# mfkiwl/conan-slam

Hardware: AMD Instinct MI355X
Metric: ekf_update_steps_per_sec (higher is better)
Workload: dtype f32

## Files before the change

conan_slam_amd/csrc/cslam_ekf.hip:

```cpp
#include <hip/hip_runtime.h>

#include <algorithm>
#include <atomic>
#include <cfloat>
#include <cmath>
#include <cstdint>
#include <cstdlib>
#include <new>
#include <string>
#include <thread>
#include <vector>

#include "cslam_common.hpp"
#include "ekf_kernels.hpp"
#include "ekf_kernels_fast.hpp"
#include "ekf_landmark_kernels.hpp"
#include "ekf_lookahead.hpp"
#include "ekf_pgemm_limbs.hpp"
#include "ekf_pose_kernels.hpp"
#include "host_linalg.hpp"

namespace cslam
{
__global__ void ekf_la_signal_kernel(unsigned* signal, unsigned add)
{
    if (threadIdx.x == 0)
    {
        atomicAdd(signal, add);
    }
}
__global__ void __launch_bounds__(128) ekf_la_wide_f32(LaWideArgs a)
{
    ekf_la_wide_body<1, 0>(a);
}
__global__ void __launch_bounds__(128) ekf_la_wide_f32_k64(LaWideArgs a)
{
    ekf_la_wide_body<1, 64>(a);
}
}

using namespace cslam;

namespace
{

std::atomic<int>& g_engines = ::cslam::live_engines();

constexpr int    kStagingSlots = 64;
constexpr size_t kLdsBudget    = 150 * 1024;

struct EkfBase
{
    virtual ~EkfBase() {}
    int         dtype    = CSLAM_F32;
    int         fuse_f64 = 1;
    int         pgemm_limbs_req = -1, limbs_kmin_req = -1;
    int         xcd_queues_req = -1;
    int         device   = 0;
    int         quirks   = CSLAM_Q_REF_EXACT;
    int         nmax     = 0;
    int         ncap     = 0;
    int         ldp      = 0;
    int         n        = 3;
    int         sync_mode = 1;
    int         seq_defer     = 1;
    int         lower         = 0;
    int         pipeline      = 0;
    int         pgemm_spare   = 16;
    int         gather_corr_wide = 1;
    int         pgemm_wgs     = 0;
    int         lookahead     = -1;
    hipStream_t stream   = nullptr;
    hipStream_t stream_b = nullptr;
    long long   la_windows = 0;

    virtual int init()                                                                        = 0;
    virtual int set_state(const void* X, int n, const void* P, int ldp)                        = 0;
    virtual int get_state(void* X, void* P, int ldp)                                           = 0;
    virtual int get_x(void* X, int cap)                                                        = 0;
    virtual int get_landmarks(int first, int count, void* x, void* pll, void* pvl)             = 0;
    virtual int trace(double* tr)                                                              = 0;
    virtual int predict(double v, double swa, const void* Q, double wb, double dt)             = 0;
    virtual int update(const void* Z, int m, const void* R, const int* idf, int batch, bool on_device) = 0;
    virtual int augment(const void* Z, int q, const void* R)                                   = 0;
    virtual int observe_heading(double phi, int use)                                           = 0;
    virtual int associate(const void* Z, int m, const void* R, double g1, double g2, int* idf_out, int* kind) = 0;
    virtual int factor_status(int* flags, int clear)                                           = 0;
    virtual int set_profiling(int on)                                                          = 0;
    virtual int get_stage_times(double* ms, int* launches)                                     = 0;
    virtual int debug_last_update(void* PHT, void* S, void* G, void* W1, void* V, int* k)      = 0;
    virtual int set_deferred(int max_cols)                                                     = 0;
    virtual int do_flush()                                                                     = 0;
    virtual int resolve_predict()                                                              = 0;
    virtual void set_fuse_predict(int on)                                                      = 0;
    virtual int sync_all()                                                                     = 0;
    virtual int la_drain()                                                                     = 0;
};

template <typename T>
struct Ekf : EkfBase
{
    T*   dX = nullptr;
    T*   dP = nullptr;
    T*   dPv = nullptr;
    T*   dWv = nullptr;
    int* dPoseDone = nullptr;
    int* dSign     = nullptr;
    T*   dLm       = nullptr;
    int  hd_cols[2] = {0, 0};
    int        wcur = 0;
    unsigned   inflight_mask = 0;
    hipEvent_t ev_a2b = nullptr, ev_pgemm = nullptr;
    T*         last_slot = nullptr;
    int  kcap  = 0;
    T*   dPHT  = nullptr;
    T*   dW1   = nullptr;
    T*   dY    = nullptr;
    int  wcap  = 0;
    int  kp    = 0;
    int  defer_max = 0;
    T*   dS    = nullptr;
    T*   dG    = nullptr;
    T*   dSub  = nullptr;
    T*   dM    = nullptr;
    bool m_valid = false;
    bool g_from_gt  = false;
    bool sub_valid = false;
    T*   dGt   = nullptr;
    T*   dV    = nullptr;
    T*   dt_   = nullptr;
    T*   dU    = nullptr;
    T*   dScrS = nullptr;
    T*   dScrG = nullptr;
    int* dFlags = nullptr;
    int* hFlags = nullptr;
    T* dHead = nullptr;
    int         mcap   = 0;
    void*       hStage = nullptr;
    void*       dStage = nullptr;
    hipEvent_t  stage_ev[kStagingSlots];
    bool        stage_ev_used[kStagingSlots];
    int         stage_next = 0;
    int*       dTicket     = nullptr;
    int        pgemm_limbs = 0;
    int        xcd_queues  = 0;
    int        limbs_kmin  = 65;
    uint4*     dWb         = nullptr;
    size_t     wb_bytes    = 0;
    int2*      dTilesM     = nullptr;
    int*       dSegOff     = nullptr;
    int*       dTicketX    = nullptr;
    int        tilesM_built = 0;
    int        limb_parity = 0;
    unsigned   launch_parity = 0;
    int        psym_nt = -1;
    int2* dTiles      = nullptr;
    int   tiles_built = 0;
    int   n_sym_tiles = 0;
    int   num_cus     = 256;
    int sticky_host = 0;
    int last_k      = 0;
    int kp_call_limit = 0;
    int                     profiling = 0;
    unsigned                prof_count = 0;
    bool                    prof_sampled = false;
    std::vector<hipEvent_t> ev_pool;
    std::vector<int>        ev_stage;
    size_t                  ev_used = 0;

    ~Ekf() override
    {
        if (stream)
        {
            (void)hipStreamSynchronize(stream);
        }
        if (stream_b && stream_b != stream)
        {
            (void)hipStreamSynchronize(stream_b);
        }
        if (stream_f)
        {
            (void)hipStreamSynchronize(stream_f);
            (void)hipEventDestroy(ev_fb);
            (void)hipEventDestroy(ev_raw);
            (void)hipStreamDestroy(stream_f);
        }
        la_free();
        if (ev_a2b)
        {
            (void)hipEventDestroy(ev_a2b);
        }
        if (ev_pgemm)
        {
            (void)hipEventDestroy(ev_pgemm);
// ... 25 lines not shown
        (void)hipFree(dSegOff);
        (void)hipFree(dTicketX);
        (void)hipFree(dPred);
        (void)hipFree(dAssoc);
        (void)hipFree(dAssocOut);
        (void)hipFree(dW1);
        (void)hipFree(dY);
        (void)hipFree(dTiles);
        (void)hipFree(dStage);
        if (hStage)
        {
            (void)hipHostFree(hStage);
        }
        if (hFlags)
        {
            (void)hipHostFree(hFlags);
        }
        if (stream_b && stream_b != stream)
        {
            (void)hipStreamDestroy(stream_b);
        }
        if (stream)
        {
            (void)hipStreamDestroy(stream);
        }
    }

    T* wbase(int region) const { return dW1 + (size_t)region * wcap * ldp; }

    void free_workspace()
    {
        (void)hipFree(dPHT);
        (void)hipFree(dS);
        (void)hipFree(dG);
        (void)hipFree(dSub);
        (void)hipFree(dM);
        dM = nullptr;
        (void)hipFree(dGt);
        (void)hipFree(dV);
        (void)hipFree(dt_);
        (void)hipFree(dU);
        (void)hipFree(dScrS);
        (void)hipFree(dScrG);
        dPHT = dS = dG = dSub = dGt = dV = dt_ = dU = dScrS = dScrG = nullptr;
    }

    int use_device() { CSLAM_HIP_TRY(hipSetDevice(device)); return CSLAM_OK; }

    int init() override
    {
        for (int i = 0; i < kStagingSlots; i++)
        {
            stage_ev_used[i] = false;
        }
        int rc = use_device();
        if (rc)
        {
            return rc;
        }
        if (xcd_queues_req >= 0)
        {
            xcd_queues = xcd_queues_req;
        }
        if (pgemm_limbs_req >= 0)
        {
            pgemm_limbs = (pgemm_limbs_req == 6 || pgemm_limbs_req == 9) ? pgemm_limbs_req : 0;
        }
        if (limbs_kmin_req >= 0)
        {
            limbs_kmin = std::max(57, limbs_kmin_req);
        }
        if (pipeline)
        {
            int lo = 0, hi = 0;
            CSLAM_HIP_TRY(hipDeviceGetStreamPriorityRange(&lo, &hi));
            CSLAM_HIP_TRY(hipStreamCreateWithPriority(&stream, hipStreamNonBlocking, hi));
            CSLAM_HIP_TRY(hipStreamCreateWithPriority(&stream_b, hipStreamNonBlocking, lo));
        }
        else
        {
            CSLAM_HIP_TRY(hipStreamCreateWithFlags(&stream, hipStreamNonBlocking));
            stream_b = stream;
        }
        CSLAM_HIP_TRY(hipEventCreateWithFlags(&ev_a2b, hipEventDisableTiming));
        CSLAM_HIP_TRY(hipEventCreateWithFlags(&ev_pgemm, hipEventDisableTiming));
        {
            hipDeviceProp_t prop;
            CSLAM_HIP_TRY(hipGetDeviceProperties(&prop, device));
            num_cus = prop.multiProcessorCount > 0 ? prop.multiProcessorCount : 256;
        }
        size_t pbytes = (size_t)ldp * ldp * sizeof(T);
        CSLAM_HIP_TRY(hipMalloc(&dX, (size_t)ldp * sizeof(T)));
        CSLAM_HIP_TRY(hipMalloc(&dP, pbytes));
        CSLAM_HIP_TRY(hipMemsetAsync(dX, 0, (size_t)ldp * sizeof(T), stream));
        CSLAM_HIP_TRY(hipMemsetAsync(dP, 0, pbytes, stream));
        CSLAM_HIP_TRY(hipMalloc(&dPv, (size_t)3 * ldp * sizeof(T)));
        CSLAM_HIP_TRY(hipMemsetAsync(dPv, 0, (size_t)3 * ldp * sizeof(T), stream));
        CSLAM_HIP_TRY(hipMalloc(&dPoseDone, 4 * sizeof(int)));
        CSLAM_HIP_TRY(hipMemsetAsync(dPoseDone, 0, 4 * sizeof(int), stream));
        CSLAM_HIP_TRY(hipMalloc(&dFlags, 2 * sizeof(int)));
        CSLAM_HIP_TRY(hipMemsetAsync(dFlags, 0, 2 * sizeof(int), stream));
        CSLAM_HIP_TRY(hipHostMalloc(&hFlags, 2 * sizeof(int), hipHostMallocDefault));
        CSLAM_HIP_TRY(hipMalloc(&dHead, ((size_t)3 * ldp + 2) * sizeof(T)));
        CSLAM_HIP_TRY(hipMemsetAsync(dHead, 0, ((size_t)3 * ldp + 2) * sizeof(T), stream));
        CSLAM_HIP_TRY(hipFuncSetAttribute(reinterpret_cast<const void*>(&ekf_factor_kernel<T>),
                                          hipFuncAttributeMaxDynamicSharedMemorySize, 160 * 1024));
        if (sizeof(T) == 4)
        {
            CSLAM_HIP_TRY(hipFuncSetAttribute(reinterpret_cast<const void*>(&ekf_factor_mfma_big_f32<128>),
                                              hipFuncAttributeMaxDynamicSharedMemorySize, 160 * 1024));
        }
        else
        {
            CSLAM_HIP_TRY(hipFuncSetAttribute(reinterpret_cast<const void*>(&ekf_factor_mfma_f64<64>),
                                              hipFuncAttributeMaxDynamicSharedMemorySize, 160 * 1024));
            CSLAM_HIP_TRY(hipFuncSetAttribute(reinterpret_cast<const void*>(&ekf_factor_mfma_f64<32>),
                                              hipFuncAttributeMaxDynamicSharedMemorySize, 160 * 1024));
            CSLAM_HIP_TRY(hipFuncSetAttribute(reinterpret_cast<const void*>(&ekf_downdate_f64<4>),
                                              hipFuncAttributeMaxDynamicSharedMemorySize, 160 * 1024));
            CSLAM_HIP_TRY(hipFuncSetAttribute(reinterpret_cast<const void*>(&ekf_downdate_f64<2>),
                                              hipFuncAttributeMaxDynamicSharedMemorySize, 160 * 1024));
        }
        CSLAM_HIP_TRY(hipMalloc(&dTicket, 2 * sizeof(int)));
        CSLAM_HIP_TRY(hipMemsetAsync(dTicket, 0, 2 * sizeof(int), stream));
        if (const char* sv = getenv("CSLAM_LA_K64"))
        {
            la_k64 = atoi(sv) ? 1 : 0;
        }
        if (const char* sv = getenv("CSLAM_LA_WG_SIGNAL"))
        {
            la_wg_signal = atoi(sv) ? 1 : 0;
        }
        if (const char* sv = getenv("CSLAM_PSYM_NT"))
        {
            psym_nt = atoi(sv) ? 1 : 0;
        }
        rc = ensure_k(64);
        if (rc)
        {
            return rc;
        }
        rc = ensure_w(128);
        if (rc)
        {
            return rc;
        }
        rc = ensure_m(64);
        if (rc)
        {
            return rc;
        }
        CSLAM_HIP_TRY(hipStreamSynchronize(stream));
        return CSLAM_OK;
    }

    int ensure_k(int k)
    {
        if (k <= kcap)
        {
            return CSLAM_OK;
        }
        int newk = round_up(std::max(k, 2 * kcap), 8);
        CSLAM_HIP_TRY(hipStreamSynchronize(stream));
        free_workspace();
        size_t pan = (size_t)ldp * newk * sizeof(T);
        size_t kk  = (size_t)newk * (newk + 1) * sizeof(T);
        CSLAM_HIP_TRY(hipMalloc(&dPHT, pan));
        CSLAM_HIP_TRY(hipMalloc(&dS, kk));
        CSLAM_HIP_TRY(hipMalloc(&dG, kk));
        if (dSub == nullptr)
        {
            CSLAM_HIP_TRY(hipMalloc(&dSub, (size_t)(3 + 64) * 64 * sizeof(T)));
            CSLAM_HIP_TRY(hipMalloc(&dM, (size_t)3 * 128 * sizeof(T)));
        }
        CSLAM_HIP_TRY(hipMalloc(&dGt, kk));
        CSLAM_HIP_TRY(hipMalloc(&dScrS, kk));
        CSLAM_HIP_TRY(hipMalloc(&dScrG, kk));
        CSLAM_HIP_TRY(hipMalloc(&dV, (size_t)newk * sizeof(T)));
        CSLAM_HIP_TRY(hipMalloc(&dt_, (size_t)newk * sizeof(T)));
        CSLAM_HIP_TRY(hipMalloc(&dU, (size_t)newk * sizeof(T)));
        CSLAM_HIP_TRY(hipMemsetAsync(dPHT, 0, pan, stream));
        (void)hipFree(dWv);
        dWv = nullptr;
        CSLAM_HIP_TRY(hipMalloc(&dWv, (size_t)3 * newk * sizeof(T)));
        CSLAM_HIP_TRY(hipMemsetAsync(dWv, 0, (size_t)3 * newk * sizeof(T), stream));
// ... 201 lines not shown
    int launch_negcol_fix(T* W, int kcols, hipStream_t st)
    {
        const int tiles = round_up(n, kTile) / kTile;
        int       rc    = CSLAM_OK;
        if (lower && (rc = ensure_tile_list(tiles)))
        {
            return rc;
        }
        const int nt = lower ? n_sym_tiles : tiles * tiles;
        hipLaunchKernelGGL(ekf_negcol_fix_kernel<T>, dim3(std::min(nt, 2 * num_cus)), dim3(256), 0, st, dP, ldp, n, W, ldp,
                           kcols, dSign + (size_t)wcur * wcap, dSign + (size_t)2 * wcap + wcur,
                           lower ? dTiles : (const int2*)nullptr, nt, tiles, dPoseDone + 2, (stream_b == stream) ? 1 : 0);
        CSLAM_HIP_TRY(hipGetLastError());
        return CSLAM_OK;
    }

    int flush_wait()
    {
        int rc = flush();
        return rc ? rc : wait_pgemm();
    }

    size_t slot_bytes(int mc) const { return (size_t)mc * (2 * sizeof(T) + sizeof(int)); }

    int ensure_m(int m)
    {
        if (m <= mcap)
        {
            return CSLAM_OK;
        }
        int newm = std::max(m, 2 * mcap);
        if (int rc = la_drain())
        {
            return rc;
        }
        CSLAM_HIP_TRY(hipStreamSynchronize(stream));
        if (stream_f)
        {
            CSLAM_HIP_TRY(hipStreamSynchronize(stream_f));
        }
        if (hStage)
        {
            (void)hipHostFree(hStage);
            hStage = nullptr;
        }
        (void)hipFree(dStage);
        dStage = nullptr;
        CSLAM_HIP_TRY(hipHostMalloc(&hStage, slot_bytes(newm) * kStagingSlots, hipHostMallocDefault));
        CSLAM_HIP_TRY(hipMalloc(&dStage, slot_bytes(newm) * kStagingSlots));
        mcap = newm;
        return CSLAM_OK;
    }

    int stage_obs(const void* Z, const int* idf, int m, bool on_device, const T** dZ, const int** dIdf)
    {
        int rc = ensure_m(m);
        if (rc)
        {
            return rc;
        }
        int slot = stage_next;
        stage_next = (stage_next + 1) % kStagingSlots;
        if (stage_ev_used[slot])
        {
            CSLAM_HIP_TRY(hipEventSynchronize(stage_ev[slot]));
        }
        else
        {
            CSLAM_HIP_TRY(hipEventCreateWithFlags(&stage_ev[slot], hipEventDisableTiming));
            stage_ev_used[slot] = true;
        }
        size_t         zb = (size_t)m * 2 * sizeof(T);
        unsigned char* ds = static_cast<unsigned char*>(dStage) + slot_bytes(mcap) * slot;
        if (on_device)
        {
            hipLaunchKernelGGL(ekf_stage_obs_kernel<T>, dim3((3 * m + 255) / 256), dim3(256), 0, stream,
                               static_cast<const T*>(Z), idf, m, reinterpret_cast<T*>(ds), reinterpret_cast<int*>(ds + zb));
            CSLAM_HIP_TRY(hipGetLastError());
        }
        else
        {
            unsigned char* hs = static_cast<unsigned char*>(hStage) + slot_bytes(mcap) * slot;
            memcpy(hs, Z, zb);
            memcpy(hs + zb, idf, (size_t)m * sizeof(int));
            CSLAM_HIP_TRY(hipMemcpyAsync(ds, hs, zb + (size_t)m * sizeof(int), hipMemcpyHostToDevice, stream));
        }
        CSLAM_HIP_TRY(hipEventRecord(stage_ev[slot], stream));
        *dZ   = reinterpret_cast<const T*>(ds);
        *dIdf = reinterpret_cast<const int*>(ds + zb);
        return CSLAM_OK;
    }

    int set_state(const void* X, int nn, const void* P, int ldph) override
    {
        if (!X || !P || nn < 3 || nn > ncap || ((nn - 3) & 1) || ldph < nn)
        {
            return fail(CSLAM_ERR_BAD_ARG, "set_state: bad n=%d (cap %d) or ldp=%d", nn, ncap, ldph);
        }
        int rc = sync_all();
        if (rc)
        {
            return rc;
        }
        CSLAM_HIP_TRY(hipMemcpyAsync(dX, X, (size_t)nn * sizeof(T), hipMemcpyHostToDevice, stream));
        CSLAM_HIP_TRY(hipMemcpy2DAsync(dP, (size_t)ldp * sizeof(T), P, (size_t)ldph * sizeof(T), (size_t)nn * sizeof(T),
                                       (size_t)nn, hipMemcpyHostToDevice, stream));
        CSLAM_HIP_TRY(hipMemcpyAsync(dPv, dP, (size_t)3 * ldp * sizeof(T), hipMemcpyDeviceToDevice, stream));
        kp        = 0;
        wcur      = 0;
        last_slot = nullptr;
        hd_cols[0] = hd_cols[1] = 0;
        CSLAM_HIP_TRY(hipMemsetAsync(dSign, 0, ((size_t)2 * wcap + 2) * sizeof(int), stream));
        CSLAM_HIP_TRY(hipMemsetAsync(dPHT, 0, (size_t)ldp * kcap * sizeof(T), stream));
        CSLAM_HIP_TRY(hipMemsetAsync(dW1, 0, (size_t)2 * ldp * wcap * sizeof(T), stream));
        CSLAM_HIP_TRY(hipStreamSynchronize(stream));
        n = nn;
        return CSLAM_OK;
    }

    int get_state(void* X, void* P, int ldph) override
    {
        if (ldph < n && P)
        {
            return fail(CSLAM_ERR_BAD_ARG, "get_state: ldp=%d < n=%d", ldph, n);
        }
        int rc = use_device();
        if (rc)
        {
            return rc;
        }
        if (P && (rc = flush_wait()))
        {
            return rc;
        }
        if (X)
        {
            CSLAM_HIP_TRY(hipMemcpyAsync(X, dX, (size_t)n * sizeof(T), hipMemcpyDeviceToHost, stream));
        }
        if (P)
        {
// ... 645 lines not shown
            {
                Gt[(size_t)r * k + c] = G[(size_t)c * k + r];
                t[c] += G[(size_t)c * k + r] * V[r];
            }
        }
        CSLAM_HIP_TRY(hipMemcpyAsync(dG, G.data(), G.size() * sizeof(T), hipMemcpyHostToDevice, stream));
        CSLAM_HIP_TRY(hipMemcpyAsync(dGt, Gt.data(), Gt.size() * sizeof(T), hipMemcpyHostToDevice, stream));
        g_from_gt  = false;
        m_valid    = false;
        CSLAM_HIP_TRY(hipMemcpyAsync(dt_, t.data(), t.size() * sizeof(T), hipMemcpyHostToDevice, stream));
        std::vector<T> u((size_t)k, (T)0);
        for (int q = 0; q < k; q++)
        {
            for (int c = 0; c < k; c++)
            {
                u[q] += G[(size_t)c * k + q] * t[c];
            }
        }
        CSLAM_HIP_TRY(hipMemcpyAsync(dU, u.data(), u.size() * sizeof(T), hipMemcpyHostToDevice, stream));
        int rc;
        if ((rc = own_region(wcur)))
        {
            return rc;
        }
        if ((rc = launch_gain(k, last_slot)))
        {
            return rc;
        }
        if (!still_pending)
        {
            const int k8 = round_up(k, 8);
            if (k8 > k)
            {
                CSLAM_HIP_TRY(hipMemset2DAsync(last_slot + (size_t)k * ldp, (size_t)ldp * sizeof(T), 0,
                                               (size_t)round_up(n, kTile) * sizeof(T), (size_t)(k8 - k), stream));
            }
            if ((rc = launch_downdate(last_slot, k, stream)))
            {
                return rc;
            }
        }
        CSLAM_HIP_TRY(hipStreamSynchronize(stream));
        return CSLAM_OK;
    }


    struct LaUpd
    {
        const T*       dZ;
        const int*     dIdf;
        int            m;
        T              R[4];
        PredictArgs<T> pp;
    };
    struct FactorOut
    {
        T *  S = nullptr, *G = nullptr, *Gt = nullptr, *V = nullptr, *t = nullptr, *U = nullptr, *M = nullptr;
        T *  sub = nullptr, *xloc = nullptr;
        int* idloc = nullptr;
    };
    LaUpd       la_q[2];
    int         la_n = 0;
    FactorOut   fo[2];
    hipStream_t stream_f = nullptr;
    hipEvent_t  ev_fb = nullptr;
    hipEvent_t  ev_raw = nullptr;
    T *         la_XL = nullptr, *la_PvL = nullptr, *la_WR = nullptr, *la_PH = nullptr, *la_PvLb = nullptr, *la_Dbb = nullptr;
    T*          la_Y = nullptr;
    LaModel<T>* la_model = nullptr;
    int         la_kpad  = 0;
    int         la_cus = 0;
    unsigned*   la_done   = nullptr;
    unsigned    la_target = 0;
    unsigned    la_seq    = 0;
    unsigned    la_sig_add = 0;
    int         la_k64 = 1;
    int         la_wg_signal = 0;

    static size_t la_chain_lds(int K)
    {
        size_t need = la_carry_lds<T>();
        if (sizeof(T) == 8)
        {
            need = std::max(need, (size_t)(K * (K + 1) + (3 + K) * (K + 1) + (K / 2) * 10 + 6 * K) * sizeof(double) +
                                      (size_t)(K / 2 + 4) * sizeof(int) + 16);
            return need;
        }
        const size_t fixed = (K == 64) ? 53984 : 15008;
        return std::max(need, (size_t)101 * 1024 - fixed);
    }
    int         la_fused   = 1;
    long long*  la_stamps  = nullptr;
    const T *dbgS = nullptr, *dbgGt = nullptr, *dbgV = nullptr;

    void la_free()
    {
        for (FactorOut& f : fo)
        {
            (void)hipFree(f.S);
            (void)hipFree(f.G);
            (void)hipFree(f.Gt);
            (void)hipFree(f.V);
            (void)hipFree(f.t);
            (void)hipFree(f.U);
            (void)hipFree(f.M);
            (void)hipFree(f.sub);
            (void)hipFree(f.xloc);
            (void)hipFree(f.idloc);
            f = FactorOut();
        }
        (void)hipFree(la_XL);
        (void)hipFree(la_PvL);
        (void)hipFree(la_WR);
        (void)hipFree(la_PH);
        (void)hipFree(la_PvLb);
        (void)hipFree(la_Dbb);
        (void)hipFree(la_Y);
        (void)hipFree(la_model);
        (void)hipFree(la_stamps);
        (void)hipFree(la_done);
        la_stamps = nullptr;
        la_done   = nullptr;
        la_XL = la_PvL = la_WR = la_PH = la_PvLb = la_Dbb = la_Y = nullptr;
        la_model = nullptr;
        la_kpad  = 0;
    }

    int la_ensure(int kp_cols)
    {
        constexpr int KM = 2 * kLaMaxObs;
        if (stream_f == nullptr)
        {
            int lo = 0, hi = 0;
            CSLAM_HIP_TRY(hipDeviceGetStreamPriorityRange(&lo, &hi));
            CSLAM_HIP_TRY(hipStreamCreateWithPriority(&stream_f, hipStreamNonBlocking, hi));
            la_cus = 1;
            CSLAM_HIP_TRY(hipEventCreateWithFlags(&ev_fb, hipEventDisableTiming));
            CSLAM_HIP_TRY(hipEventCreateWithFlags(&ev_raw, hipEventDisableTiming));
            CSLAM_HIP_TRY(hipFuncSetAttribute(reinterpret_cast<const void*>(&ekf_la_chain_kernel<T, 32>),
                                              hipFuncAttributeMaxDynamicSharedMemorySize, (int)la_chain_lds(32)));
            CSLAM_HIP_TRY(hipFuncSetAttribute(reinterpret_cast<const void*>(&ekf_la_chain_kernel<T, 64>),
                                              hipFuncAttributeMaxDynamicSharedMemorySize, (int)la_chain_lds(64)));
            CSLAM_HIP_TRY(hipMalloc(&la_done, 768 * sizeof(unsigned)));
            CSLAM_HIP_TRY(hipMemset(la_done, 0, 768 * sizeof(unsigned)));
            la_target = 0;
            la_seq    = 0;
            for (FactorOut& f : fo)
            {
                CSLAM_HIP_TRY(hipMalloc(&f.S, (size_t)KM * (KM + 1) * sizeof(T)));
                CSLAM_HIP_TRY(hipMalloc(&f.G, (size_t)KM * (KM + 1) * sizeof(T)));
                CSLAM_HIP_TRY(hipMalloc(&f.Gt, (size_t)KM * (KM + 1) * sizeof(T)));
                CSLAM_HIP_TRY(hipMalloc(&f.V, (size_t)KM * sizeof(T)));
                CSLAM_HIP_TRY(hipMalloc(&f.t, (size_t)KM * sizeof(T)));
                CSLAM_HIP_TRY(hipMalloc(&f.U, (size_t)KM * sizeof(T)));
                CSLAM_HIP_TRY(hipMalloc(&f.M, (size_t)3 * KM * sizeof(T)));
                CSLAM_HIP_TRY(hipMalloc(&f.sub, (size_t)(3 + KM) * KM * sizeof(T)));
                CSLAM_HIP_TRY(hipMalloc(&f.xloc, (size_t)(3 + KM) * sizeof(T)));
                CSLAM_HIP_TRY(hipMalloc(&f.idloc, (size_t)kLaMaxObs * sizeof(int)));
            }
            CSLAM_HIP_TRY(hipMalloc(&la_XL, (size_t)2 * KM * sizeof(T)));
            CSLAM_HIP_TRY(hipMalloc(&la_PvL, (size_t)2 * KM * 3 * sizeof(T)));
            CSLAM_HIP_TRY(hipMalloc(&la_PH, (size_t)KM * KM * sizeof(T)));
            CSLAM_HIP_TRY(hipMalloc(&la_PvLb, (size_t)KM * 3 * sizeof(T)));
            CSLAM_HIP_TRY(hipMalloc(&la_Dbb, (size_t)KM * KM * sizeof(T)));
            CSLAM_HIP_TRY(hipMalloc(&la_Y, (size_t)KM * KM * sizeof(T)));
            CSLAM_HIP_TRY(hipMalloc(&la_model, 2 * sizeof(LaModel<T>)));
            if (const char* fv = getenv("CSLAM_LA_FUSED"))
            {
                la_fused = atoi(fv) ? 1 : 0;
            }
            if (getenv("CSLAM_LA_STAMPS"))
            {
                CSLAM_HIP_TRY(hipMalloc(&la_stamps, 32 * sizeof(long long)));
                CSLAM_HIP_TRY(hipMemset(la_stamps, 0, 32 * sizeof(long long)));
            }
        }
        if (kp_cols > la_kpad)
        {
            CSLAM_HIP_TRY(hipStreamSynchronize(stream));
            CSLAM_HIP_TRY(hipStreamSynchronize(stream_f));
            (void)hipFree(la_WR);
            la_WR   = nullptr;
            la_kpad = 0;
            const int kpad = round_up(std::max(kp_cols, 128), 64);
            CSLAM_HIP_TRY(hipMalloc(&la_WR, (size_t)2 * KM * kpad * sizeof(T)));
            la_kpad = kpad;
        }
        return CSLAM_OK;
    }

    bool la_eligible(int m) const
    {
        const int k = 2 * m;
        const bool on = lookahead > 0 || (lookahead < 0 && sizeof(T) == 4 && n >= 7000 && g_engines.load() == 1);
        return on && !sync_mode && !pipeline && profiling != 1 && k > 16 && k <= 2 * kLaMaxObs && gather_corr_wide &&
               fuse_predict && (sizeof(T) == 4 || fuse_f64) && defer_max >= k + (la_n ? 2 * la_q[0].m : k) &&
               wcap >= k + (la_n ? 2 * la_q[0].m : k) && seq.count == 0 && hd_cols[0] == 0 && hd_cols[1] == 0 && n > 3 &&
               kp_call_limit == 0;
    }

    int la_enqueue(const T* dZ, const int* dIdf, int m, const T* R, bool on_device)
    {
        if (on_device && la_n == 0)
        {
            if (int rc = stage_obs(dZ, dIdf, m, true, &dZ, &dIdf))
            {
                return rc;
            }
        }
        LaUpd u;
        u.dZ   = dZ;
        u.dIdf = dIdf;
        u.m    = m;
        for (int i = 0; i < 4; i++)
        {
            u.R[i] = R[i];
        }
        u.pp     = pp;
        pp.valid = 0;
        la_q[la_n++] = u;
        return la_n == 2 ? la_launch_window() : CSLAM_OK;
    }

    FactorArgs<T> la_factor_args(const LaUpd& u, FactorOut& f)
    {
        FactorArgs<T> a;
        a.X   = f.xloc;
        a.n   = 3 + 2 * u.m;
        a.Z   = u.dZ;
        a.idf = fo[0].idloc;
        a.m   = u.m;
        for (int i = 0; i < 4; i++)
        {
            a.R[i] = u.R[i];
        }
        a.PHT      = dPHT;
        a.ldw      = ldp;
        a.dS       = f.S;
        a.dG       = f.G;
        a.dGt      = f.Gt;
        a.dV       = f.V;
        a.dt       = f.t;
        a.flags    = dFlags;
        a.scratchS = dScrS;
        a.scratchG = dScrG;
        a.textbook = (quirks & CSLAM_Q_LOWER_CHOL_GAIN) ? 0 : 1;
        a.stamps   = (la_stamps && &f == &fo[0]) ? la_stamps : nullptr;
        a.sub      = f.sub;
        a.dM       = f.M;
        a.pp       = PredictArgs<T>{0, (T)0, (T)0, (T)0, (T)0, (T)0, (T)0, (T)0, (T)0, 0};
        a.P3       = dPv;
        a.ldp3     = ldp;
        a.pred_out = nullptr;
        a.lds_S    = 1;
        a.lds_G    = 1;
        return a;
    }

    int la_wide(const LaUpd& u, const FactorOut& f, hipEvent_t ev_factor)
    {
        const int k = 2 * u.m;
        pp          = u.pp;
        fuse_now    = pp.valid != 0;
// ... 22 lines not shown
        CSLAM_HIP_TRY(hipGetLastError());
        if (ev_factor != nullptr)
        {
            CSLAM_HIP_TRY(hipStreamWaitEvent(stream, ev_factor, 0));
        }
        T*  slot = wbase(wcur) + (size_t)kp * ldp;
        int rc   = launch_gain(k, slot, f.Gt, f.U, f.M);
        if (rc)
        {
            return rc;
        }
        pp.valid  = 0;
        fuse_now  = false;
        last_slot = slot;
        kp += k;
        dbgS      = f.S;
        dbgGt     = f.Gt;
        dbgV      = f.V;
        g_from_gt = true;
        sub_valid = false;
        return CSLAM_OK;
    }

    int la_launch_window()
    {
        const int nu = la_n;
        if (nu == 0)
        {
            return CSLAM_OK;
        }
        la_n = 0;
        const LaUpd ua = la_q[0], ub = la_q[1];
        const PredictArgs<T> held = pp;
        int rc = use_device();
        if (rc)
        {
            return rc;
        }
        const int ka = 2 * ua.m, kb = nu == 2 ? 2 * ub.m : 0;
        if (kp > 256 && (rc = flush()))
        {
            return rc;
        }
        if ((rc = ensure_k(2 * kLaMaxObs)) || (rc = ensure_w(ka + kb)) || (rc = la_ensure(kp)))
        {
            return rc;
        }
        if (lower && (rc = ensure_tile_list(round_up(n, kTile) / kTile)))
        {
            return rc;
        }
        const bool     safe     = g_engines.load() > 1;
        const unsigned n_blocks = (unsigned)(3 + ka + 2 * kb);
        auto launch_chain = [&]() -> int {
            LaChainArgs<T> ch;
            ch.fa   = la_factor_args(ua, fo[0]);
            ch.fb   = la_factor_args(nu == 2 ? ub : ua, fo[1]);
            ch.du_a = fo[0].U;
            ch.du_b = fo[1].U;
            ch.nu   = nu;
            ch.done = la_done;
            ch.target  = la_target + n_blocks;
            ch.timeout = 20000000ull;
            ch.chain_done = la_done + 256;
            ch.seq        = ++la_seq;
            LaCarryArgs<T>& ca = ch.ca;
            ca.n       = n;
            ca.m_a     = ua.m;
            ca.m_b     = nu == 2 ? ub.m : 0;
            ca.idf_b   = nu == 2 ? ub.dIdf : ua.dIdf;
            ca.pp_b    = nu == 2 ? ub.pp : ua.pp;
            ca.PH      = la_PH;
            ca.Dbb     = la_Dbb;
            ca.PvLb    = la_PvLb;
            ca.XLb     = la_XL + ka;
            ca.model_a = la_model;
            ca.Gt_a    = fo[0].Gt;
            ca.u_a     = fo[0].U;
            ca.M_a     = fo[0].M;
            ca.sub_a   = fo[0].sub;
            ca.sub_b   = fo[1].sub;
            ca.xloc_b  = fo[1].xloc;
            ca.model_b = la_model + 1;
            ca.Y_b     = la_Y;
            if (std::max(ka, kb) <= 32)
            {
                hipLaunchKernelGGL((ekf_la_chain_kernel<T, 32>), dim3(1), dim3(256), la_chain_lds(32), stream_f, ch);
            }
            else
            {
                hipLaunchKernelGGL((ekf_la_chain_kernel<T, 64>), dim3(1), dim3(256), la_chain_lds(64), stream_f, ch);
            }
            CSLAM_HIP_TRY(hipGetLastError());
            CSLAM_HIP_TRY(hipEventRecord(ev_fb, stream_f));
            return CSLAM_OK;
        };
        if (!safe && (rc = launch_chain()))
        {
            return rc;
        }
        const T* Wp = wbase(wcur);
        LaRowsArgs<T> ra;
        ra.X     = dX;
        ra.Pv    = dPv;
        ra.ldp   = ldp;
        ra.n     = n;
        ra.idf_a = ua.dIdf;
        ra.ra    = ka;
        ra.idf_b = nu == 2 ? ub.dIdf : ua.dIdf;
        ra.rb    = kb;
        ra.Wp    = Wp;
        ra.ldw   = ldp;
        ra.kp    = kp;
        ra.kpad  = la_kpad;
        ra.XL    = la_XL;
        ra.PvL   = la_PvL;
        ra.WR    = la_WR;
        ra.flags = dFlags;
        hipLaunchKernelGGL(ekf_la_rows_kernel<T>, dim3(ka + kb), dim3(128), 0, stream, ra);
        LaPrepArgs<T> pa;
        pa.P       = dP;
        pa.ldp     = ldp;
        pa.n       = n;
        pa.lower   = lower;
        pa.X       = dX;
        pa.Pv      = dPv;
        pa.idf_a   = ua.dIdf;
        pa.idf_b   = nu == 2 ? ub.dIdf : ua.dIdf;
        pa.ra      = ka;
        pa.rb      = kb;
        pa.pp_a    = ua.pp;
        pa.XL      = la_XL;
        pa.PvL     = la_PvL;
        pa.WR      = la_WR;
        pa.kp      = kp;
        pa.kpad    = la_kpad;
        pa.sub_a   = fo[0].sub;
        pa.PH      = la_PH;
        pa.Dbb     = la_Dbb;
        pa.PvLb    = la_PvLb;
        pa.model_a = la_model;
        pa.xloc_a  = fo[0].xloc;
        pa.idloc   = fo[0].idloc;
        const int  k8f      = round_up(kp, 8);
        const bool pg_signal = !la_wg_signal && !safe && kp > 0 && seq.count == 0 && sizeof(T) == 4 && k8f <= 128 && lower && ldp < 32768 &&
                               !limbs_take(k8f) && stream_b == stream && hd_cols[wcur] == 0;
        pa.done    = pg_signal ? (unsigned*)nullptr : la_done;
        hipLaunchKernelGGL(ekf_la_blocks_kernel<T>, dim3(n_blocks), dim3(64), 0, stream, pa);
        CSLAM_HIP_TRY(hipGetLastError());
        if (safe)
        {
            CSLAM_HIP_TRY(hipEventRecord(ev_raw, stream));
            CSLAM_HIP_TRY(hipStreamWaitEvent(stream_f, ev_raw, 0));
            if ((rc = launch_chain()))
            {
                return rc;
            }
        }
        la_target += n_blocks;
        la_sig_add = pg_signal ? n_blocks : 0u;
        rc         = flush();
        if (la_sig_add != 0)
        {
            const unsigned add = la_sig_add;
            la_sig_add         = 0;
            hipLaunchKernelGGL(ekf_la_signal_kernel, dim3(1), dim3(64), 0, stream, la_done, add);
        }
        if (rc)
        {
            return rc;
        }
        bool fused = false;
        if constexpr (std::is_same<T, float>::value)
        {
            if (la_fused)
            {
                fused = true;
                if (safe)
                {
                    CSLAM_HIP_TRY(hipStreamWaitEvent(stream, ev_fb, 0));
                }
                LaWideArgs wa;
                wa.chain_done = la_done + 256;
                wa.seq        = la_seq;
                wa.timeout    = 20000000ull;
                wa.flags      = dFlags;
                wa.stamps     = la_stamps ? la_stamps + 16 : nullptr;
                wa.wg_times   = nullptr;
                wa.P       = dP;
                wa.ldp     = ldp;
                wa.n       = n;
                wa.lower   = getenv("CSLAM_LA_TIMING_DIRECT") ? 0 : lower;
                wa.X       = dX;
                wa.Pv      = dPv;
                wa.nu      = nu;
                wa.idf_a   = ua.dIdf;
                wa.idf_b   = nu == 2 ? ub.dIdf : ua.dIdf;
                wa.ma      = ua.m;
                wa.mb      = nu == 2 ? ub.m : 0;
                wa.valid_a = ua.pp.valid;
// ... 796 lines not shown

int cslam_ekf_augment(cslam_ekf_t h, const void* Z, int q, const void* R)
{
    CSLAM_NEED(h);
    if (int rc = B(h)->resolve_predict())
    {
        return rc;
    }
    return B(h)->augment(Z, q, R);
}

int cslam_ekf_associate(cslam_ekf_t h, const void* Z, int m, const void* R, double gate1, double gate2, int* idf_out,
                        int* kind_out)
{
    CSLAM_NEED(h);
    if (int rc = B(h)->resolve_predict())
    {
        return rc;
    }
    return B(h)->associate(Z, m, R, gate1, gate2, idf_out, kind_out);
}

int cslam_ekf_observe_heading(cslam_ekf_t h, double phi, int use_heading)
{
    CSLAM_NEED(h);
    return B(h)->observe_heading(phi, use_heading);
}

int cslam_ekf_set_pgemm_workgroups(cslam_ekf_t h, int workgroups)
{
    CSLAM_NEED(h);
    if (workgroups < 0)
    {
        return fail(CSLAM_ERR_BAD_ARG, "set_pgemm_workgroups: negative");
    }
    B(h)->pgemm_wgs = workgroups;
    return CSLAM_OK;
}

int cslam_ekf_lookahead_windows(cslam_ekf_t h, long long* windows)
{
    CSLAM_NEED(h);
    if (!windows)
    {
        return fail(CSLAM_ERR_BAD_ARG, "lookahead_windows: null");
    }
    *windows = B(h)->la_windows;
    return CSLAM_OK;
}

int cslam_ekf_get_streams(cslam_ekf_t h, void** chain_stream, void** pgemm_stream)
{
    CSLAM_NEED(h);
    if (chain_stream)
    {
        *chain_stream = reinterpret_cast<void*>(B(h)->stream);
    }
    if (pgemm_stream)
    {
        *pgemm_stream = reinterpret_cast<void*>(B(h)->stream_b);
    }
    return CSLAM_OK;
}

int cslam_ekf_run_many(cslam_ekf_t* handles, int count, int steps, const double* v, const double* swa, const void* Q,
                       double wb, double dt, const void* const* dZ, const int* const* d_idf, int m, const void* R,
                       int batch)
{
    if (!handles || count < 0 || steps < 0 || m < 0 || !R || !Q || (steps > 0 && (!v || !swa)) || (m > 0 && (!dZ || !d_idf)))
    {
        return fail(CSLAM_ERR_BAD_ARG, "run_many: bad arguments");
    }
    for (int i = 0; i < count; i++)
    {
        if (!handles[i] || (m > 0 && (!dZ[i] || !d_idf[i])))
        {
            return fail(CSLAM_ERR_BAD_ARG, "run_many: null handle or input for instance %d", i);
        }
    }
    std::vector<int>         rcs((size_t)count, CSLAM_OK);
    std::vector<std::string> msgs((size_t)count);
    auto                     body = [&](int i) {
        EkfBase*     e     = B(handles[i]);
        const size_t esz   = (e->dtype == CSLAM_F32) ? sizeof(float) : sizeof(double);
        const char*  zbase = m > 0 ? static_cast<const char*>(dZ[i]) : nullptr;
        for (int t = 0; t < steps; t++)
        {
            int rc = e->predict(v[t], swa[t], Q, wb, dt);
            if (!rc && m > 0)
            {
                rc = e->update(zbase + (size_t)t * 2 * m * esz, m, R, d_idf[i] + (size_t)t * m, batch, true);
            }
            if (rc)
            {
                rcs[(size_t)i]  = rc;
                msgs[(size_t)i] = last_error_buf();
                return;
            }
        }
    };
    if (count == 1)
    {
        body(0);
    }
    else
    {
// ... 65 lines not shown
```

conan_slam_amd/csrc/ekf_kernels.hpp:

```cpp
#pragma once

#include <hip/hip_runtime.h>

#include "device_math.hpp"

namespace cslam
{

constexpr int kFlagLltFailed = 1;
constexpr int kFlagZeroed    = 2;
constexpr int kFlagBadIdf    = 8;
constexpr int kFlagHeadingSkipped = 32;

__device__ inline int clamp_idf(int idf, int n)
{
    const int nf = (n - 3) >> 1;
    return idf < 1 ? 1 : (idf > nf ? (nf > 0 ? nf : 1) : idf);
}

typedef float  f32x16 __attribute__((ext_vector_type(16)));
typedef double f64x4 __attribute__((ext_vector_type(4)));

template <typename T>
struct Vec4;
// ... 561 lines not shown
    {
        const int  j     = base + lane;
        const bool valid = j < nf;
        const T*   f     = feat + (size_t)(valid ? j : 0) * 8;
        const T    v0    = z0 - f[5];
        const T    v1    = pi2pi<T>(z1 - f[6]);
        const T    t0    = v0 * f[0] + v1 * f[1];
        const T    t1    = v0 * f[2] + v1 * f[3];
        const T    nis   = t0 * v0 + t1 * v1;
        const T    nd    = nis + f[4];
        const bool gated = valid && (nis < gate1);
        const T    cand  = (gated && nd == nd) ? nd : inf;
        T incl = cand;
#pragma unroll
        for (int dlt = 1; dlt < 64; dlt <<= 1)
        {
            const T up = __shfl_up(incl, dlt);
            if (lane >= dlt)
            {
                incl = (up < incl) ? up : incl;
            }
        }
        T excl = __shfl_up(incl, 1);
        excl   = (lane == 0) ? inf : excl;
        const T    before = (nbest < excl) ? nbest : excl;
        const bool record = gated && (nd < before);
        if (valid && !record && nis < outer)
        {
            outer = nis;
        }
        const T cmin = __shfl(incl, 63);
        if (cmin < nbest)
        {
            const unsigned long long hits = __ballot(cand == cmin);
            jbest                         = base + __builtin_ctzll(hits) + 1;
            nbest                         = cmin;
        }
    }
#pragma unroll
    for (int dlt = 32; dlt >= 1; dlt >>= 1)
    {
        const T o = __shfl_xor(outer, dlt);
        outer     = (o < outer) ? o : outer;
    }
    if (lane == 0)
    {
        idf_out[i] = jbest;
        kind[i]    = (jbest != 0) ? 1 : ((outer > gate2) ? 2 : 0);
    }
}

template <typename T>
__global__ void __launch_bounds__(256) ekf_stage_obs_kernel(const T* __restrict__ Z, const int* __restrict__ idf, int m,
                                                             T* __restrict__ Zs, int* __restrict__ idfs)
{
    const int i = blockIdx.x * 256 + threadIdx.x;
    if (i < 2 * m)
    {
        Zs[i] = Z[i];
    }
    else if (i < 3 * m)
    {
        idfs[i - 2 * m] = idf[i - 2 * m];
    }
}

template <typename T>
__global__ void __launch_bounds__(256) ekf_pending_y_kernel(const T* __restrict__ X, int n, const T* __restrict__ Z,
                                                             const int* __restrict__ idf, int m,
                                                             const T* __restrict__ Wp, int ldw, int kp,
                                                             T* __restrict__ Y, const int* __restrict__ sgn = nullptr)
{
    __shared__ T   s_coef[10];
    __shared__ int s_fx;
    const int      o = blockIdx.x;
    if (threadIdx.x == 0)
    {
        T v[2];
        observe_model<T>(X, n, idf[o], Z[2 * o], Z[2 * o + 1], s_coef, v, &s_fx);
    }
    __syncthreads();
    const int q = blockIdx.y * 256 + threadIdx.x;
    if (q >= kp)
    {
        return;
    }
    const T* w  = Wp + (size_t)q * ldw;
    const int fx = s_fx;
    const T  w0 = w[0], w1 = w[1], w2 = w[2], wa = w[fx], wb = w[fx + 1];
    T        y0 = s_coef[0] * w0;
    y0 += s_coef[1] * w1;
    y0 += s_coef[2] * w2;
    y0 += s_coef[3] * wa;
    y0 += s_coef[4] * wb;
    T y1 = s_coef[5] * w0;
    y1 += s_coef[6] * w1;
    y1 += s_coef[7] * w2;
    y1 += s_coef[8] * wa;
    y1 += s_coef[9] * wb;
    const int k = 2 * m;
    if (sgn != nullptr && sgn[q] != 0)
    {
        y0 = -y0;
        y1 = -y1;
    }
    Y[(size_t)q * k + 2 * o]     = y0;
    Y[(size_t)q * k + 2 * o + 1] = y1;
}

constexpr int kCorrChunk = 64;

template <typename T>
__global__ void __launch_bounds__(256) ekf_pending_corr_kernel(int n, int m, const T* __restrict__ Wp, int ldw, int kp,
                                                                const T* __restrict__ Y, T* __restrict__ PHT,
                                                                int ldpht)
{
// ... 507 lines not shown
```

conan_slam_amd/csrc/ekf_lookahead.hpp:

```cpp
#pragma once

#include <hip/hip_runtime.h>

#include "ekf_kernels.hpp"
#include "ekf_kernels_fast.hpp"

namespace cslam
{

constexpr int kLaMaxObs = 32;

__device__ inline int la_row(const int* __restrict__ idf, int s, int n)
{
    return 3 + 2 * clamp_idf(idf[s >> 1], n) - 2 + (s & 1);
}

template <typename T>
struct LaRowsArgs
{
    const T* X;
    const T* Pv;
    int      ldp, n;
    const int* idf_a;
    int        ra;
    const int* idf_b;
    int        rb;
    const T*   Wp;
    int        ldw, kp, kpad;
    T *        XL, *PvL, *WR;
    int*       flags;
};

template <typename T>
__device__ __forceinline__ void ekf_la_rows_body(const LaRowsArgs<T>& a)
{
    const T* __restrict__ X = a.X;
    const T* __restrict__ Pv = a.Pv;
    const int ldp = a.ldp, n = a.n, ra = a.ra, rb = a.rb, ldw = a.ldw, kp = a.kp;
    const int* __restrict__ idf_a = a.idf_a;
    const int* __restrict__ idf_b = a.idf_b;
    const T* __restrict__ Wp = a.Wp;
    T* __restrict__ XL = a.XL;
    T* __restrict__ PvL = a.PvL;
    T* __restrict__ WR = a.WR;
    int* __restrict__ flags = a.flags;

    const int s   = blockIdx.x;
    if (threadIdx.x == 4)
    {
        const int id = (s < ra) ? idf_a[s >> 1] : idf_b[(s - ra) >> 1];
        if (id < 1 || id > ((n - 3) >> 1))
        {
            atomicOr(&flags[0], kFlagBadIdf);
        }
    }
    const int row = (s < ra) ? la_row(idf_a, s, n) : la_row(idf_b, s - ra, n);
    for (int q = threadIdx.x; q < kp; q += 128)
    {
        WR[(size_t)q * 128 + s] = Wp[(size_t)q * ldw + row];
    }
    if (threadIdx.x < 3)
    {
        PvL[s * 3 + threadIdx.x] = Pv[(size_t)threadIdx.x * ldp + row];
    }
    if (threadIdx.x == 3)
    {
        XL[s] = X[row];
    }
}

template <typename T>
__global__ void __launch_bounds__(128) ekf_la_rows_kernel(LaRowsArgs<T> a)
{
    ekf_la_rows_body<T>(a);
}


template <typename T>
struct LaModel
{
    T g02, g12;
    T pose[3];
    T pvv[9];
    T coef[kLaMaxObs * 10];
    T pad[2];
};

template <typename T>
__device__ inline void la_predict_row(const PredictArgs<T>& pp, T g02, T g12, int row, T* a)
{
    if (pp.valid && row - 3 < pp.w)
    {
        T o0, o1, o2;
        predict_stripe_col<T>(g02, g12, a[0], a[1], a[2], &o0, &o1, &o2);
        a[0] = o0;
        a[1] = o1;
        a[2] = o2;
    }
}

template <typename T>
__device__ inline void la_predict_pose(const PredictArgs<T>& pp, const T* pose_in, const T* pvv_in, T* pose, T* g, T* pvv)
{
    pose[0] = pose_in[0], pose[1] = pose_in[1], pose[2] = pose_in[2];
    g[0] = g[1] = (T)0;
    for (int e = 0; e < 9; e++)
    {
        pvv[e] = pvv_in[e];
    }
    if (pp.valid)
    {
        predicted_pose<T>(pp, pose_in, &pose[0], &pose[1], &pose[2]);
        predict_gv<T>(pp, pose_in[2], &g[0], &g[1]);
        predict_pvv<T>(pp, pose_in[2], pvv_in, pvv);
    }
}

template <typename T>
__device__ inline void la_pht_pair(const T* c, T p0, T p1, T p2, T pa, T pb, T* v0, T* v1)
{
    T s0 = p0 * c[0];
    s0 += p1 * c[1];
    s0 += p2 * c[2];
    s0 += pa * c[3];
    s0 += pb * c[4];
    T s1 = p0 * c[5];
// ... 480 lines not shown
    }
    if (tid < mb)
    {
        T   v[2];
        int fx;
        observe_model_pose<T>(xl, 3 + kb, tid + 1, (T)0, (T)0, xl[0], xl[1], xl[2], &coef[tid * 10], v, &fx);
    }
    __syncthreads();
    for (int e = tid; e < (3 + kb) * mb; e += 256)
    {
        const int slot = e / mb, o = e % mb;
        const T*  br   = &blk[slot * LB];
        T         v0, v1;
        la_pht_pair<T>(&coef[o * 10], br[0], br[1], br[2], br[3 + 2 * o], br[3 + 2 * o + 1], &v0, &v1);
        a.sub_b[slot * kb + 2 * o]     = v0;
        a.sub_b[slot * kb + 2 * o + 1] = v1;
    }
    for (int e = tid; e < ka * mb; e += 256)
    {
        const int q = e / mb, o = e % mb;
        const T*  c = &coef[o * 10];
        const T   wa = w1t[q * LD + 2 * o], wb = w1t[q * LD + 2 * o + 1];
        T         y0 = c[3] * wa;
        y0 += c[4] * wb;
        T y1 = c[8] * wa;
        y1 += c[9] * wb;
        a.Y_b[(size_t)q * kb + 2 * o]     = y0;
        a.Y_b[(size_t)q * kb + 2 * o + 1] = y1;
    }
    for (int e = tid; e < 3 + kb; e += 256)
    {
        a.xloc_b[e] = xl[e];
    }
    LaModel<T>& mo = *a.model_b;
    if (tid == 0)
    {
        mo.g02 = s_g[0];
        mo.g12 = s_g[1];
    }
    if (tid < 3)
    {
        mo.pose[tid] = xl[tid];
    }
    if (tid < 9)
    {
        mo.pvv[tid] = s_pvv[tid];
    }
    for (int e = tid; e < mb * 10; e += 256)
    {
        mo.coef[e] = coef[e];
    }
}

constexpr int kFlagLaTimeout = 16;

template <typename T>
struct LaChainArgs
{
    FactorArgs<T>   fa, fb;
    T *             du_a, *du_b;
    LaCarryArgs<T>  ca;
    int             nu;
    const unsigned* done;
    unsigned        target;
    unsigned long long timeout;
    unsigned*       chain_done;
    unsigned        seq;
};

template <typename T, int K>
__device__ __forceinline__ void ekf_la_chain_body(const LaChainArgs<T>& a)
{
    extern __shared__ __align__(16) unsigned char la_chain_smem[];
    if (threadIdx.x < 64)
    {
        const unsigned long long t0 = __builtin_amdgcn_s_memrealtime();
        while (true)
        {
            unsigned c = threadIdx.x < 16
                             ? __hip_atomic_load(a.done + 16 * threadIdx.x, __ATOMIC_RELAXED, __HIP_MEMORY_SCOPE_AGENT)
                             : 0u;
            c += __shfl_xor(c, 1);
            c += __shfl_xor(c, 2);
            c += __shfl_xor(c, 4);
            c += __shfl_xor(c, 8);
            c = __shfl(c, 0);
            if ((int)(c - a.target) >= 0)
            {
                break;
            }
            __builtin_amdgcn_s_sleep(32);
            if (__builtin_amdgcn_s_memrealtime() - t0 > a.timeout)
            {
                if (threadIdx.x == 0)
                {
                    atomicOr(&a.fa.flags[0], kFlagLaTimeout);
                }
                break;
            }
        }
    }
    __syncthreads();
    __builtin_amdgcn_fence(__ATOMIC_ACQUIRE, "agent");
    if constexpr (std::is_same<T, float>::value)
    {
        ekf_factor_mfma_f32_body<K>(a.fa, a.du_a);
    }
// ... 647 lines not shown
```

Baseline: 13200.

## Stage lookahead observations on side stream with device-side flag wait

Device-side observation staging for lookahead updates now runs on the secondary stream_f instead of the main stream. The consumer rows kernel spins on a per-slot sequence word in device memory, or the stream waits on an event when multiple engines are active. This takes the staging copy off the critical path of the main chain stream so it can overlap with prior work. In exchange it adds spin-wait and timeout logic, extra per-slot flag words, and a window-reuse guard on staging slots.

```diff
diff --git a/conan_slam_amd/csrc/cslam_ekf.hip b/conan_slam_amd/csrc/cslam_ekf.hip
--- a/conan_slam_amd/csrc/cslam_ekf.hip
+++ b/conan_slam_amd/csrc/cslam_ekf.hip
@@ -73,6 +73,7 @@
     hipStream_t stream   = nullptr;
     hipStream_t stream_b = nullptr;
     long long   la_windows = 0;
+    bool        streams_exposed = false;
 
     virtual int init()                                                                        = 0;
     virtual int set_state(const void* X, int n, const void* P, int ldp)                        = 0;
@@ -140,6 +141,8 @@
     void*       dStage = nullptr;
     hipEvent_t  stage_ev[kStagingSlots];
     bool        stage_ev_used[kStagingSlots];
+    long long   stage_win[kStagingSlots];
+    unsigned    stage_seq = 0;
     int         stage_next = 0;
     int*       dTicket     = nullptr;
     int        pgemm_limbs = 0;
@@ -271,6 +274,7 @@
         for (int i = 0; i < kStagingSlots; i++)
         {
             stage_ev_used[i] = false;
+            stage_win[i]     = -2;
         }
         int rc = use_device();
         if (rc)
@@ -350,6 +354,10 @@
         {
             la_wg_signal = atoi(sv) ? 1 : 0;
         }
+        if (const char* sv = getenv("CSLAM_LA_PREP"))
+        {
+            la_prep = atoi(sv) ? 1 : 0;
+        }
         if (const char* sv = getenv("CSLAM_PSYM_NT"))
         {
             psym_nt = atoi(sv) ? 1 : 0;
@@ -657,7 +665,7 @@
         return CSLAM_OK;
     }
 
-    int stage_obs(const void* Z, const int* idf, int m, bool on_device, const T** dZ, const int** dIdf)
+    int stage_obs(const void* Z, const int* idf, int m, bool on_device, const T** dZ, const int** dIdf, int* f_slot = nullptr)
     {
         int rc = ensure_m(m);
         if (rc)
@@ -677,10 +685,18 @@
         }
         size_t         zb = (size_t)m * 2 * sizeof(T);
         unsigned char* ds = static_cast<unsigned char*>(dStage) + slot_bytes(mcap) * slot;
+        const bool    on_f   = f_slot != nullptr && 3 * m <= 256 && la_windows >= stage_win[slot] + 2;
+        hipStream_t   st     = on_f ? stream_f : stream;
+        if (f_slot != nullptr)
+        {
+            *f_slot = on_f ? slot : -1;
+        }
+        stage_win[slot] = la_windows;
         if (on_device)
         {
-            hipLaunchKernelGGL(ekf_stage_obs_kernel<T>, dim3((3 * m + 255) / 256), dim3(256), 0, stream,
-                               static_cast<const T*>(Z), idf, m, reinterpret_cast<T*>(ds), reinterpret_cast<int*>(ds + zb));
+            hipLaunchKernelGGL(ekf_stage_obs_kernel<T>, dim3((3 * m + 255) / 256), dim3(256), 0, st,
+                               static_cast<const T*>(Z), idf, m, reinterpret_cast<T*>(ds), reinterpret_cast<int*>(ds + zb),
+                               on_f ? la_done + kLaStageWords + 16 * slot : (unsigned*)nullptr, on_f ? ++stage_seq : 0u);
             CSLAM_HIP_TRY(hipGetLastError());
         }
         else
@@ -690,7 +706,7 @@
             memcpy(hs + zb, idf, (size_t)m * sizeof(int));
             CSLAM_HIP_TRY(hipMemcpyAsync(ds, hs, zb + (size_t)m * sizeof(int), hipMemcpyHostToDevice, stream));
         }
-        CSLAM_HIP_TRY(hipEventRecord(stage_ev[slot], stream));
+        CSLAM_HIP_TRY(hipEventRecord(stage_ev[slot], st));
         *dZ   = reinterpret_cast<const T*>(ds);
         *dIdf = reinterpret_cast<const int*>(ds + zb);
         return CSLAM_OK;
@@ -1442,6 +1458,8 @@
         int            m;
         T              R[4];
         PredictArgs<T> pp;
+        int            f_slot;
+        unsigned       f_seq;
     };
     struct FactorOut
     {
@@ -1466,6 +1484,8 @@
     unsigned    la_sig_add = 0;
     int         la_k64 = 1;
     int         la_wg_signal = 0;
+    int         la_prep = 1;
+    static constexpr int kLaStageWords = 768, kLaWords = 768 + 16 * kStagingSlots;
 
     static size_t la_chain_lds(int K)
     {
@@ -1531,10 +1551,11 @@
                                               hipFuncAttributeMaxDynamicSharedMemorySize, (int)la_chain_lds(32)));
             CSLAM_HIP_TRY(hipFuncSetAttribute(reinterpret_cast<const void*>(&ekf_la_chain_kernel<T, 64>),
                                               hipFuncAttributeMaxDynamicSharedMemorySize, (int)la_chain_lds(64)));
-            CSLAM_HIP_TRY(hipMalloc(&la_done, 768 * sizeof(unsigned)));
-            CSLAM_HIP_TRY(hipMemset(la_done, 0, 768 * sizeof(unsigned)));
+            CSLAM_HIP_TRY(hipMalloc(&la_done, kLaWords * sizeof(unsigned)));
+            CSLAM_HIP_TRY(hipMemset(la_done, 0, kLaWords * sizeof(unsigned)));
             la_target = 0;
             la_seq    = 0;
+            stage_seq = 0;
             for (FactorOut& f : fo)
             {
                 CSLAM_HIP_TRY(hipMalloc(&f.S, (size_t)KM * (KM + 1) * sizeof(T)));
@@ -1591,14 +1612,19 @@
 
     int la_enqueue(const T* dZ, const int* dIdf, int m, const T* R, bool on_device)
     {
+        int      f_slot = -1;
         if (on_device && la_n == 0)
         {
-            if (int rc = stage_obs(dZ, dIdf, m, true, &dZ, &dIdf))
+            const bool try_f = la_prep && !streams_exposed && g_engines.load() == 1;
+            int        rc    = try_f ? la_ensure(0) : CSLAM_OK;
+            if (rc || (rc = stage_obs(dZ, dIdf, m, true, &dZ, &dIdf, try_f ? &f_slot : nullptr)))
             {
                 return rc;
             }
         }
         LaUpd u;
+        u.f_slot = f_slot;
+        u.f_seq  = stage_seq;
         u.dZ   = dZ;
         u.dIdf = dIdf;
         u.m    = m;
@@ -1727,6 +1753,11 @@
         }
         const bool     safe     = g_engines.load() > 1;
         const unsigned n_blocks = (unsigned)(3 + ka + 2 * kb);
+        const bool rows_wait = ua.f_slot >= 0 && !safe;
+        if (ua.f_slot >= 0 && !rows_wait)
+        {
+            CSLAM_HIP_TRY(hipStreamWaitEvent(stream, stage_ev[ua.f_slot], 0));
+        }
         auto launch_chain = [&]() -> int {
             LaChainArgs<T> ch;
             ch.fa   = la_factor_args(ua, fo[0]);
@@ -1792,7 +1823,6 @@
         ra.PvL   = la_PvL;
         ra.WR    = la_WR;
         ra.flags = dFlags;
-        hipLaunchKernelGGL(ekf_la_rows_kernel<T>, dim3(ka + kb), dim3(128), 0, stream, ra);
         LaPrepArgs<T> pa;
         pa.P       = dP;
         pa.ldp     = ldp;
@@ -1821,6 +1851,12 @@
         const bool pg_signal = !la_wg_signal && !safe && kp > 0 && seq.count == 0 && sizeof(T) == 4 && k8f <= 128 && lower && ldp < 32768 &&
                                !limbs_take(k8f) && stream_b == stream && hd_cols[wcur] == 0;
         pa.done    = pg_signal ? (unsigned*)nullptr : la_done;
+        LaStageWait sw;
+        sw.word    = rows_wait ? la_done + kLaStageWords + 16 * ua.f_slot : (const unsigned*)nullptr;
+        sw.seq     = ua.f_seq;
+        sw.timeout = 20000000ull;
+        sw.flags   = dFlags;
+        hipLaunchKernelGGL(ekf_la_rows_kernel<T>, dim3(ka + kb), dim3(128), 0, stream, ra, sw);
         hipLaunchKernelGGL(ekf_la_blocks_kernel<T>, dim3(n_blocks), dim3(64), 0, stream, pa);
         CSLAM_HIP_TRY(hipGetLastError());
         if (safe)
@@ -2723,6 +2759,7 @@
 int cslam_ekf_get_streams(cslam_ekf_t h, void** chain_stream, void** pgemm_stream)
 {
     CSLAM_NEED(h);
+    B(h)->streams_exposed = true;
     if (chain_stream)
     {
         *chain_stream = reinterpret_cast<void*>(B(h)->stream);
diff --git a/conan_slam_amd/csrc/ekf_kernels.hpp b/conan_slam_amd/csrc/ekf_kernels.hpp
--- a/conan_slam_amd/csrc/ekf_kernels.hpp
+++ b/conan_slam_amd/csrc/ekf_kernels.hpp
@@ -637,7 +637,8 @@
 
 template <typename T>
 __global__ void __launch_bounds__(256) ekf_stage_obs_kernel(const T* __restrict__ Z, const int* __restrict__ idf, int m,
-                                                             T* __restrict__ Zs, int* __restrict__ idfs)
+                                                             T* __restrict__ Zs, int* __restrict__ idfs,
+                                                             unsigned* word, unsigned seq)
 {
     const int i = blockIdx.x * 256 + threadIdx.x;
     if (i < 2 * m)
@@ -647,6 +648,15 @@
     else if (i < 3 * m)
     {
         idfs[i - 2 * m] = idf[i - 2 * m];
+    }
+    if (word != nullptr)
+    {
+        __builtin_amdgcn_fence(__ATOMIC_RELEASE, "agent");
+        __syncthreads();
+        if (threadIdx.x == 0)
+        {
+            __hip_atomic_store(word, seq, __ATOMIC_RELAXED, __HIP_MEMORY_SCOPE_AGENT);
+        }
     }
 }
 
diff --git a/conan_slam_amd/csrc/ekf_lookahead.hpp b/conan_slam_amd/csrc/ekf_lookahead.hpp
--- a/conan_slam_amd/csrc/ekf_lookahead.hpp
+++ b/conan_slam_amd/csrc/ekf_lookahead.hpp
@@ -69,9 +69,41 @@
     }
 }
 
+constexpr int kFlagLaTimeout = 16;
+
+struct LaStageWait
+{
+    const unsigned* word;
+    unsigned        seq;
+    unsigned long long timeout;
+    int*            flags;
+};
+
+__device__ __forceinline__ void la_wait_word(const LaStageWait& w)
+{
+    const unsigned long long t0 = __builtin_amdgcn_s_memrealtime();
+    while ((int)(__hip_atomic_load(w.word, __ATOMIC_RELAXED, __HIP_MEMORY_SCOPE_AGENT) - w.seq) < 0)
+    {
+        __builtin_amdgcn_s_sleep(2);
+        if (__builtin_amdgcn_s_memrealtime() - t0 > w.timeout)
+        {
+            if ((threadIdx.x & 63) == 0)
+            {
+                atomicOr(&w.flags[0], kFlagLaTimeout);
+            }
+            break;
+        }
+    }
+    __builtin_amdgcn_fence(__ATOMIC_ACQUIRE, "agent");
+}
+
 template <typename T>
-__global__ void __launch_bounds__(128) ekf_la_rows_kernel(LaRowsArgs<T> a)
-{
+__global__ void __launch_bounds__(128) ekf_la_rows_kernel(LaRowsArgs<T> a, LaStageWait w)
+{
+    if (w.word != nullptr)
+    {
+        la_wait_word(w);
+    }
     ekf_la_rows_body<T>(a);
 }
 
@@ -658,7 +690,6 @@
     }
 }
 
-constexpr int kFlagLaTimeout = 16;
 
 template <typename T>
 struct LaChainArgs
```

Result: no change. 13190 (-0.0%).
